# openai/tiktoken

Measured on AMD Instinct MI355X. Metric: GB/s text encoded (o200k_base-shaped vocab, 1 GiB corpus per GPU), bit-exact vs CoreBPE restatement, higher is better.
Workload: dtype u8; 1 GPU; o200k_shaped encode_ordinary_batch, 1024 MiB synthetic web-text per GPU (tkc_generate mix=1, seed 0x5EED0003), 318404 docs on rank 0, inputs resident in HBM, packed u32 output; encoding=o200k_shaped, pat_str_runs_on=hand-written scanners, bytes_per_gpu=1073741824, docs_rank0=318404, rccl_ranks=0, devices_visible=1, pieces_rank0=162498410, parallelism=doc-sharded x1

## Files before the change

### tiktoken_amd/csrc/tk_api.hip

```cpp
#include <hip/hip_runtime.h>
#include <dlfcn.h>
#include <rccl/rccl.h>
#include <stdio.h>
#include <stdlib.h>
#include <string.h>

#include <chrono>
#include <functional>
#include <algorithm>
#include <array>
#include <atomic>
#include <map>
#include <memory>
#include <mutex>
#include <string>
#include <thread>
#include <utility>
#include <vector>

#include "../../include/tiktoken_amd.h"
#include "tk_decode.h"
#include "tk_offsets.h"
#include "tk_rows.h"
#include "tk_train.h"
// ... 78 lines not shown
        std::swap(p, o.p);
        return *this;
    }
    ~HostResult() { if (p) tk_free(p); }
    T* release() { return std::exchange(p, nullptr); }
    operator T*() const { return p; }
};

struct KernelStat {
    double ms = 0;
    uint64_t launches = 0;
};

#define TK_NAUX 6
#define TK_NSET 4

#define TK_WORK_BUFS(X)                                                                                                                                  \
    X(text_al) X(tile_sum) X(wide_ws) X(scan_sums) X(row_base) X(brk) X(docb) X(cand) X(ss) X(si) X(starts) X(blockcnt) X(pstart) X(res) X(staging)     \
    X(listB) X(listC) X(counters) X(total) X(g_id) X(g_rk) X(g_nx) X(g_pv) X(g_lv) X(tile_np) X(tile_nt) X(mt_keys) X(mtab) X(movf) X(mcnt) X(wbin)       \
    X(deferred) X(big) X(rx_spec) X(rx_gst) X(rx_lnk) X(rx_exit) X(merge_work) X(find)
struct WorkSet {
    Pinned<uint32_t> h_counters;
    Pinned<uint64_t> h_total;
    Stream sb;
    Event ev_front;
    Event ev_cnt;
    Event ev_tot;
    Event ev_done;
    Event ev_fork, ev_join[TK_NAUX];
#define X(name) Buf name;
    TK_WORK_BUFS(X)
#undef X
    uint64_t bytes() const {
        uint64_t t = 0;
#define X(name) t += name.cap;
        TK_WORK_BUFS(X)
#undef X
        return t;
    }
};
#define TK_GROW (-1000)
#define TK_RESYNC (-1001)
#define TK_SPEC_HIT (-1002)
#ifndef TK_MT_DIV
#define TK_MT_DIV 128
#endif
// ... 35 lines not shown
    uint32_t ovf_base = 0;
    uint32_t ovf_cap = 0;
    bool optimistic = false;
};

static TkMiss miss_of(WorkSet& w, const ChunkJob& job) { return TkMiss{w.mtab.as<TkMissTab>(), w.movf.as<TkMissOvf>(), job.ovf_base, w.mcnt.as<uint8_t>()}; }

struct tk_core {
    int device = 0;
    Stream stream;
    Stream aux[TK_NAUX];
    Stream cs_h2d, cs_d2h;
    Pinned<void> stage[2];
    Event ev_stage[2];
    TkHostTables H;
    TkTables D;
    Buf t_stage1, t_stage2, t_bmp, t_byte_tab, t_short, t_mid, t_dec, t_piece, t_piece_off, t_tok_bytes, t_pair, t_pair2, t_byte_rank, t_xl, t_xfilter, t_spec_bytes, t_spec_off, t_spec_id, t_spec_head;
    uint32_t spec_max_len = 0;
    bool has_rx = false;
    bool has_rx_fb = false;
    TkRxCompiled rx_fb;
    uint64_t st_fallbacks = 0;
    uint64_t st_regrown = 0;
    uint64_t st_resynced = 0;
    bool defer_sync = false;
    uint32_t defer_ppm = 1u << 12;
    TkRxDev rx{};
    Buf t_rx_ins, t_rx_sets, t_rx_ranges, t_rx_first, t_rx_s1, t_rx_s2, t_rx_dtrans, t_rx_dascii, t_rx_ds1, t_rx_ds2;
    int rx_form = TK_RX_FORM_PROGRAM;
    std::mutex mu;
    WorkSet ws[TK_NSET];
    Buf text, doc_off, out_tokens, out_tok_off, allowed, tok_bases;
    Buf disallowed;
    bool find_on = false;
    uint64_t find_hit = ~0ull;
    uint64_t st_find_launches = 0;
    hipStream_t back_for = nullptr;
    struct BackChoice {
        hipStream_t s[3];
        int n;
    };
    std::map<hipStream_t, BackChoice> back_known;
    bool back_probed = false;
    hipStream_t back_s[3] = {};
    int n_back = 0;
    Pinned<uint32_t> h_probe;
// ... 159 lines not shown
    }
    int ndev = 0;
    if (hipGetDeviceCount(&ndev) != hipSuccess || ndev <= 0)
        return fail(TK_RUNTIME_ERROR, "no HIP device available: tiktoken_amd has no CPU path");
    if (device < 0 || device >= ndev) return fail(TK_VALUE_ERROR, "device ordinal out of range");
    struct Destroy {
        void operator()(tk_core* core) const { tk_destroy(core); }
    };
    std::unique_ptr<tk_core, Destroy> owner(new tk_core());
    tk_core* c = owner.get();
    c->device = device;
    std::string err = tk_build_tables(ranks_blob, ranks_off, ranks_ids, n_ranks, spec_blob, spec_off, spec_ids, n_spec, pat_str, &c->H);
    if (!err.empty()) return fail(TK_VALUE_ERROR, err);
    if (hipSetDevice(device) != hipSuccess) return fail(TK_RUNTIME_ERROR, "hipSetDevice failed");
    if (c->stream.create() != hipSuccess) return fail(TK_RUNTIME_ERROR, "hipStreamCreate failed");
    for (int i = 0; i < TK_NAUX; ++i)
        if (c->aux[i].create() != hipSuccess) return fail(TK_RUNTIME_ERROR, "hipStreamCreate failed");
    for (WorkSet& w : c->ws) {
        if (w.sb.create() != hipSuccess) return fail(TK_RUNTIME_ERROR, "hipStreamCreate failed");
        for (Event* e : {&w.ev_front, &w.ev_cnt, &w.ev_tot, &w.ev_done, &w.ev_fork})
            if (e->create() != hipSuccess) return fail(TK_RUNTIME_ERROR, "hipEventCreate failed");
        for (int i = 0; i < TK_NAUX; ++i)
            if (w.ev_join[i].create() != hipSuccess) return fail(TK_RUNTIME_ERROR, "hipEventCreate failed");
        if (w.h_counters.alloc(2 * TK_CNT_N * 4 + 64, hipHostMallocDefault) != hipSuccess || w.h_total.alloc(64, hipHostMallocDefault) != hipSuccess)
            return fail(TK_RUNTIME_ERROR, "hipHostMalloc failed");
    }
    const TkHostTables& H = c->H;
    auto upload_rx = [&](const TkRxCompiled& X) -> int {
        TRY(upload(c->t_rx_ins, X.ins.data(), X.ins.size() * sizeof(TkRxIns)));
        TRY(upload(c->t_rx_sets, X.sets.data(), X.sets.size() * sizeof(TkRxSet)));
        TRY(upload(c->t_rx_ranges, X.ranges.data(), X.ranges.size() * 4));
        TRY(upload(c->t_rx_first, X.first.data(), X.first.size() * 4));
        TRY(upload(c->t_rx_s1, tk_rx_props_stage1(), 0x1100));
        TRY(upload(c->t_rx_s2, tk_rx_props_stage2(), (size_t)tk_rx_props_blocks() * 256));
        c->rx = TkRxDev{c->t_rx_ins.as<TkRxIns>(), c->t_rx_sets.as<TkRxSet>(), c->t_rx_ranges.as<uint32_t>(), c->t_rx_s1.as<uint8_t>(),
                        c->t_rx_s2.as<uint8_t>(), (uint32_t)X.ins.size(), (uint32_t)X.sets.size(), (uint32_t)X.ranges.size() / 2,
                        c->t_rx_first.as<uint32_t>(), (uint32_t)X.first.size() / 8, nullptr, nullptr, nullptr, nullptr, 0u, 0u, 0u};
        c->rx_form = TK_RX_FORM_PROGRAM;
        const char* want = getenv("TIKTOKEN_AMD_RX_MATCHER");
        if (X.has_dfa() && !(want && !strcmp(want, "program"))) {
            std::vector<uint16_t> tr(X.dfa_trans);
            tr.resize((tr.size() + 1) & ~(size_t)1, 0);
            TRY(upload(c->t_rx_dtrans, tr.data(), tr.size() * 2));
            TRY(upload(c->t_rx_dascii, X.dfa_ascii.data(), 384));
            TRY(upload(c->t_rx_ds1, X.dfa_s1.data(), X.dfa_s1.size() * 2));
            TRY(upload(c->t_rx_ds2, X.dfa_s2.data(), X.dfa_s2.size()));
            c->rx.dfa_trans = c->t_rx_dtrans.as<uint16_t>();
            c->rx.dfa_ascii = c->t_rx_dascii.as<uint8_t>();
// ... 161 lines not shown
    uint64_t g = (items + per_block - 1) / per_block;
    if (g < 1) g = 1;
    if (g > cap) g = cap;
    return (uint32_t)g;
}

template <int MODE>
static void launch_front(tk_core* c, const ChunkJob& job, dim3 grid, hipStream_t s, uint32_t* deferred, int internal_dbg) {
    const ChunkAsk& a = job.ask;
    const FrontArgs& f = job.front;
    auto go = [&](auto* kernel) {
        hipLaunchKernelGGL(kernel, grid, dim3(256), 0, s, c->D, a.d_text, a.n, a.base, f.brk, f.docb, f.ss, f.si, f.out, f.mt, f.mt_mask, deferred, f.gapb, f.dbg | internal_dbg);
    };
    auto of_pattern = [&](auto pat) {
        if (f.ss) go(tk_k_front<decltype(pat)::value, true, MODE>);
        else go(tk_k_front<decltype(pat)::value, false, MODE>);
    };
    if (f.pat_id == TK_PAT_R50K) of_pattern(std::integral_constant<int, TK_PAT_R50K>{});
    else if (f.pat_id == TK_PAT_CL100K) of_pattern(std::integral_constant<int, TK_PAT_CL100K>{});
    else if (f.pat_id == TK_PAT_O200K) of_pattern(std::integral_constant<int, TK_PAT_O200K>{});
    else of_pattern(std::integral_constant<int, TK_PAT_GENERIC>{});
}

static int scan_u32(tk_core* c, WorkSet& w, hipStream_t s, uint32_t* a, uint64_t n, uint64_t* total_out) {
    if (n <= 2 * (uint64_t)TK_SCAN_BLOCK) {
        TRY(timed(c, s, "tk_k_scan_small", [&] { hipLaunchKernelGGL(tk_k_scan_small, dim3(1), dim3(TK_SCAN_THREADS), 0, s, a, n, total_out); }));
        return TK_OK;
    }
    const uint64_t nb = (n + TK_SCAN_BLOCK - 1) / TK_SCAN_BLOCK;
    TRY(ensure(w.scan_sums, (nb + 2) * 4));
    uint32_t* sums = w.scan_sums.as<uint32_t>();
    TRY(timed(c, s, "tk_k_scan_sums", [&] { hipLaunchKernelGGL(tk_k_scan_sums, dim3((uint32_t)nb), dim3(TK_SCAN_THREADS), 0, s, a, n, sums); }));
    TRY(timed(c, s, "tk_k_scan_small", [&] { hipLaunchKernelGGL(tk_k_scan_small, dim3(1), dim3(TK_SCAN_THREADS), 0, s, sums, nb, total_out); }));
    TRY(timed(c, s, "tk_k_scan_apply", [&] { hipLaunchKernelGGL(tk_k_scan_apply, dim3((uint32_t)nb), dim3(TK_SCAN_THREADS), 0, s, a, n, sums); }));
    return TK_OK;
}

static int rx_failure(const uint32_t* counters, uint64_t base) {
    const std::string at = std::to_string(base + (uint64_t)(~counters[TK_CNT_RXPOS]));
    if (counters[TK_CNT_ERR] & TK_RX_ERR_STACK)
        return fail(TK_VALUE_ERROR, "pat_str: a repeated group needs more backtracking state than the matcher keeps (piece at byte " + at +
                                        " of the batch); make the group possessive, e.g. (?:...)++");
    return fail(TK_VALUE_ERROR, "pat_str: backtrack limit exceeded at byte " + at +
                                    " of the batch (nested quantifiers; the reference's fancy-regex gives up after 1 000 000 backtracks as well)");
}

struct RxPairs {
    const uint64_t nwords;
    explicit RxPairs(uint64_t n) : nwords((n + 31) / 32) {}
    uint64_t bytes() const { return 2 * (nwords + 2) * 4; }
    uint32_t* gap(const Buf& pair) const { return pair.as<uint32_t>() + nwords + 2; }
    static std::array<Buf*, 3> of(WorkSet& w) { return {&w.rx_spec, &w.rx_gst, &w.rx_lnk}; }
};

static int rx_split(tk_core* c, WorkSet& w, const ChunkJob& job, hipStream_t s) {
    const uint8_t* d_text = job.ask.d_text;
    const uint64_t n = job.ask.n, nwords = (n + 31) / 32;
// ... 118 lines not shown
    TRY(ensure(w.big, (1 + 3 * TK_BIGCOPY_CAP) * 4));
    TkClearArgs clr;
    clr.n = 0;
    auto clear = [&](Buf& b, uint64_t bytes, uint32_t v) -> int {
        TRY(ensure(b, bytes));
        clr.p[clr.n] = b.as<uint4>();
        clr.n16[clr.n] = (bytes + 15) / 16;
        clr.v[clr.n] = v;
        ++clr.n;
        return TK_OK;
    };
    TRY(clear(w.brk, (nwords + 2) * 4, 0u));
    TRY(clear(w.counters, TK_CNT_N * 4, 0u));
    TRY(clear(w.big, 4, 0u));
    TRY(clear(w.merge_work, 16 * TKM_WORK_STRIDE * 4, 0u));
    TRY(clear(w.total, 32, 0u));
    uint32_t* find_docb = nullptr;
    const bool docs_in_place = n > 0 && !single_piece && ask.d_tok_off != nullptr;
    TRY(ensure(w.row_base, (ntiles + 4) * 4));
    if (docs_in_place) TRY(clear(w.row_base, (ntiles + 2) * 4, 0xFFFFFFFFu));
    TRY(clear(w.tile_sum, ntiles + 16, 0xFFFFFFFFu));
    FrontArgs& f = job.front;
    if (job.ovf_base) {
        TRY(clear(w.mt_keys, sizeof(TkMissKey) * job.ovf_base, 0xFFFFFFFFu));
        job.mt = w.mt_keys.as<TkMissKey>();
    }
    f.pat_id = T.pat.generic() ? TK_PAT_GENERIC : T.pattern;
    f.brk = w.brk.as<uint32_t>();
    f.out = TkFrontOut{w.starts.as<uint32_t>(), w.tile_np.as<uint32_t>(), w.res.as<uint32_t>(), w.tile_sum.as<uint8_t>(), miss_of(w, job), job.ovf_cap, w.listC.as<uint32_t>(), w.counters.as<uint32_t>()};
    f.mt = (c->dbg & TK_DBG_NO_MT) ? (TkMissKey*)nullptr : job.mt;
    f.mt_mask = (1u << job.mt_bits) - 1u;
    f.dbg = (c->dbg & ~TK_DBG_INTERNAL) | (pretok_only ? TK_DBG_STARTS_ONLY : 0);
    if (n > 0 && !single_piece) {
        if (ask.use_special) {
            for (Buf* b : {&w.docb, &w.cand}) TRY(clear(*b, (nwords + 4) * 4, 0u));
            for (Buf* b : {&w.ss, &w.si}) TRY(clear(*b, (nwords + 2) * 4, 0u));
            f.docb = w.docb.as<uint32_t>();
            f.ss = w.ss.as<uint32_t>();
            f.si = w.si.as<uint32_t>();
        }
        if (c->find_on && !pretok_only) {
            job.find = true;
            TRY(clear(w.find, 16, 0xFFFFFFFFu));
            if (!f.docb) TRY(clear(w.docb, (nwords + 4) * 4, 0u));
            find_docb = w.docb.as<uint32_t>();
        }
        if (c->has_rx) {
// ... 27 lines not shown
        }
        if (c->has_rx) TRY(rx_split(c, w, job, s));
        TRY(ensure(w.deferred, 2 * (ntiles + 2) * 4));
        TRY(timed(c, s, "tk_k_front", [&] {
            launch_front<TKF_MODE_TILE>(c, job, dim3((uint32_t)ntiles), s, w.deferred.as<uint32_t>(), (c->has_rx && !(c->dbg & TK_DBG_SCANNERS)) ? TK_DBG_HARD_ONLY : 0);
        }));
    } else if (n > 0) {
        hipLaunchKernelGGL(tk_k_chunk_clear, dim3(1), dim3(256), 0, s, clr);
        clr.n = 0;
        TRY(timed(c, s, "tk_k_single_front", [&] { hipLaunchKernelGGL(tk_k_single_front, dim3(1), dim3(64), 0, s, T, d_text, (uint32_t)n, f.out, ask.kind == ChunkKind::SinglePieceNoLookup ? 1 : 0); }));
    }
    if (clr.n) hipLaunchKernelGGL(tk_k_chunk_clear, dim3(1), dim3(256), 0, s, clr);
    HIPCHK(hipEventRecord(w.ev_front, s));
    return TK_OK;
}

static int piece_starts(tk_core* c, WorkSet& w, const ChunkJob& job, hipStream_t s, uint64_t* count_out) {
    const uint64_t n = job.ask.n, nwords = (n + 31) / 32, nblk = (nwords + 255) / 256;
    uint32_t *starts = w.starts.as<uint32_t>(), *blockcnt = w.blockcnt.as<uint32_t>();
    uint64_t P = 0;
    TRY(ensure(w.pstart, 16));
    if (n > 0) {
        TRY(timed(c, s, "tk_k_count", [&] { hipLaunchKernelGGL(tk_k_count, dim3((uint32_t)nblk), dim3(256), 0, s, starts, nwords, blockcnt); }));
        TRY(timed(c, s, "tk_k_scan_small", [&] { hipLaunchKernelGGL(tk_k_scan_small, dim3(1), dim3(TK_SCAN_THREADS), 0, s, blockcnt, nblk, w.total.as<uint64_t>()); }));
        HIPCHK(hipMemcpyAsync(&P, w.total.p, 8, hipMemcpyDeviceToHost, s));
        HIPCHK(hipStreamSynchronize(s));
        if (w.h_counters[TK_CNT_ERR] & (TK_RX_ERR_GAP | TK_RX_ERR_STACK | TK_RX_ERR_LIMIT)) return rx_failure(w.h_counters, job.ask.base);
        TRY(ensure(w.pstart, (P + 2) * 4));
        TRY(timed(c, s, "tk_k_emit", [&] {
            hipLaunchKernelGGL(tk_k_emit, dim3((uint32_t)nblk), dim3(256), 0, s, starts, nwords, blockcnt, w.pstart.as<uint32_t>(), P, n, job.front.gapb);
        }));
    } else {
        HIPCHK(hipMemsetAsync(w.pstart.p, 0, 4, s));
    }
    *count_out = P;
    return TK_OK;
}

static int stage_back(tk_core* c, WorkSet& w, ChunkJob& job, hipStream_t s, hipEvent_t prev_tot = nullptr) {
    const TkTables& T = c->D;
    const ChunkAsk& ask = job.ask;
    const uint64_t n = ask.n, ntiles = job.ntiles;
    const uint8_t* d_text = ask.d_text;
    uint32_t *d_out = ask.d_out, *counters = w.counters.as<uint32_t>();
    uint32_t *res = w.res.as<uint32_t>(), *stg = w.staging.as<uint32_t>();
    const TkMiss data = miss_of(w, job);
    uint32_t *tile_np = w.tile_np.as<uint32_t>(), *tile_nt = w.tile_nt.as<uint32_t>();
// ... 79 lines not shown
            if (rounds) {
                TRY(timed(c, s, "tk_k_merge_rounds", [&] {
                    hipLaunchKernelGGL(tk_k_merge_rounds, dim3(grid_for(nC, 1, 1024)), dim3(TKB_THREADS), 0, s, T, d_text, w.listC.as<uint32_t>(),
                                       (uint32_t)nC, w.g_id.as<uint32_t>(), w.g_rk.as<uint32_t>(), w.g_nx.as<uint32_t>(), w.g_pv.as<uint32_t>(),
                                       data, stg);
                }));
            }
            if (rounds && n >= TK_WIDE_MIN) {
                TRY(ensure(w.wide_ws, sizeof(TkWideWs)));
                HIPCHK(hipMemsetAsync(w.wide_ws.p, 0, sizeof(TkWideWs), s));
                TRY(timed(c, s, "tk_k_merge_rounds_wide", [&] {
                    hipLaunchKernelGGL(tk_k_merge_rounds_wide, dim3(TK_WIDE_BLOCKS), dim3(TKB_THREADS), 0, s, T, d_text, w.listC.as<uint32_t>(),
                                       (uint32_t)nC, w.g_id.as<uint32_t>(), w.g_rk.as<uint32_t>(), w.g_nx.as<uint32_t>(), w.g_pv.as<uint32_t>(),
                                       data, stg, w.wide_ws.as<TkWideWs>());
                }));
            }
            TRY(timed(c, s, "tk_k_merge_long", [&] {
                hipLaunchKernelGGL(tk_k_merge_long, dim3(grid_for(nC, 4, 8192)), dim3(256), 0, s, T, d_text, w.listC.as<uint32_t>(), (uint32_t)nC,
                                   w.g_id.as<uint32_t>(), w.g_rk.as<uint32_t>(), w.g_nx.as<uint32_t>(), w.g_pv.as<uint32_t>(),
                                   w.g_lv.as<uint64_t>(), data, stg, rounds ? 1 : 0);
            }));
        }
    }
    const bool small_rows = n < (8u << 20);
    if (encode) {
        TRY(timed(c, s, "tk_k_count_tiles", [&] {
            if (small_rows) hipLaunchKernelGGL(tk_k_count_tiles<1>, dim3(grid_for(ntiles, 4, 2048)), dim3(256), 0, s, ntiles, tile_np, res, data, tile_nt,
                               w.total.as<unsigned long long>());
            else hipLaunchKernelGGL(tk_k_count_tiles<TKP_ROWS_COUNT>, dim3(grid_for(ntiles, 4, 2048)), dim3(256), 0, s, ntiles, tile_np, res, data, tile_nt,
                               w.total.as<unsigned long long>());
        }));
        TRY(scan_u32(c, w, s, tile_nt, ntiles, w.total.as<uint64_t>()));
    } else {
        HIPCHK(hipMemsetAsync(w.total.p, 0, 32, s));
    }
    if (prev_tot) HIPCHK(hipStreamWaitEvent(s, prev_tot, 0));
    hipLaunchKernelGGL(tk_k_advance, dim3(1), dim3(64), 0, s, c->tok_bases.as<unsigned long long>(), job.index, w.total.as<uint64_t>());
    HIPCHK(hipEventRecord(w.ev_tot, s));
    if (encode) {
        TRY(timed(c, s, "tk_k_place", [&] {
            const bool docs_in_place = !ask.single_piece() && ask.d_tok_off != nullptr;
            const TkPlaceDocs docs{ask.d_doc_off, ask.base, n, ask.n_docs, w.row_base.as<uint32_t>(), w.starts.as<uint32_t>(), w.total.as<uint64_t>(), docs_in_place ? ask.d_tok_off : (uint64_t*)nullptr};
            hipLaunchKernelGGL(tk_k_place<TKP_ROWS_PLACE>, dim3(grid_for(ntiles, 4, 6144)), dim3(256), 0, s, ntiles, tile_np, tile_nt, res, data, stg, d_out, tok_base, w.big.as<uint32_t>(), docs);
        }));
    }
    if (encode && n > TK_BIGCOPY)
        hipLaunchKernelGGL(tk_k_bigcopy, dim3(1024), dim3(256), 0, s, w.big.as<uint32_t>(), stg, d_out, tok_base);
    if (!front_only && ask.d_tok_off && (n == 0 || ask.single_piece())) {
        TRY(timed(c, s, "tk_k_docoff", [&] {
            hipLaunchKernelGGL(tk_k_docoff, dim3(grid_for(ask.n_docs + 1, 16, 4096)), dim3(256), 0, s, ask.n_docs, ask.d_doc_off, ask.base, n, w.starts.as<uint32_t>(), tile_nt, res, data,
                               (n > 0 && !ask.single_piece()) ? w.row_base.as<uint32_t>() : (const uint32_t*)nullptr, w.total.as<uint64_t>(), tok_base, ask.d_tok_off);
        }));
    }
    HIPCHK(hipMemcpyAsync(w.h_total, w.total.p, 16, hipMemcpyDeviceToHost, s));
    if (job.find) HIPCHK(hipMemcpyAsync(w.h_total + 2, w.find.p, 8, hipMemcpyDeviceToHost, s));
    HIPCHK(hipMemcpyAsync(w.h_counters + TK_CNT_N, counters, TK_CNT_N * 4, hipMemcpyDeviceToHost, s));
    HIPCHK(hipEventRecord(w.ev_done, s));
    c->st_long += nC;
    return TK_OK;
}

static int chunk_finish(tk_core* c, WorkSet& w, const ChunkJob& job, uint64_t* n_tokens_out) {
    HIPCHK(hipEventSynchronize(w.ev_done));
    if (job.find && w.h_total[2] != ~0ull) {
        c->find_hit = w.h_total[2];
        return TK_SPEC_HIT;
    }
    const uint32_t* hb = w.h_counters + TK_CNT_N;
    uint64_t nB = 0;
    for (int b = 0; b < TK_NBIN; ++b) {
        nB += hb[TK_CNT_BIN0 + b];
        if ((c->dbg & TK_DBG_VERBOSE) && hb[TK_CNT_BIN0 + b]) fprintf(stderr, "bin %d (%u..%u bytes): %u pieces\n", b, tk_bin_lo(b), tk_bin_hi(b), hb[TK_CNT_BIN0 + b]);
    }
    if (hb[TK_CNT_ERR] & (TK_RX_ERR_GAP | TK_RX_ERR_STACK | TK_RX_ERR_LIMIT)) return rx_failure(hb, job.ask.base);
    if (hb[TK_CNT_ERR]) return fail(TK_RUNTIME_ERROR, "internal error in the front kernel (scanner list overflow, code " + std::to_string(hb[TK_CNT_ERR]) + ")");
    if (job.optimistic) {
        if (hb[TK_CNT_DEFER2]) {
            c->defer_sync = true;
            return TK_RESYNC;
        }
        const uint32_t ppm = (uint32_t)std::min<uint64_t>(((uint64_t)hb[TK_CNT_DEFER] << 20) / (job.ntiles ? job.ntiles : 1), 1u << 20);
        c->defer_ppm = std::max(ppm, c->defer_ppm / 4);
    }
    if (hb[TK_CNT_OVF] > job.ovf_cap && !job.ask.piece_starts()) {
        c->ovf_full = true;
        return TK_GROW;
    }
    c->st_bytes += job.ask.n;
    c->st_pieces += w.h_total[1];
    c->st_tokens += w.h_total[0];
    c->st_medium += nB;
    c->st_chunks += 1;
    *n_tokens_out = w.h_total[0];
    return TK_OK;
}

static int run_chunk(tk_core* c, hipStream_t s, const ChunkAsk& ask, uint64_t* n_out) {
    WorkSet& w = c->ws[0];
    ChunkJob job;
    TRY(ensure(c->tok_bases, 64));
    HIPCHK(hipMemsetAsync(c->tok_bases.p, 0, 16, s));
    TRY(stage_front(c, w, job, s, ask));
    if (ask.piece_starts()) {
        TRY(stage_deferred(c, w, job, s));
        return piece_starts(c, w, job, s, n_out);
    }
    TRY(stage_back(c, w, job, s));
    return chunk_finish(c, w, job, n_out);
}

static int prepare_mask(tk_core* c, hipStream_t s, Buf& mask, const uint32_t* ids, uint64_t n, bool* any) {
    const TkHostTables& H = c->H;
    std::vector<uint8_t> a(H.spec_id.size() + 16, 0);
    *any = false;
    for (size_t k = 0; k < H.spec_id.size(); ++k)
// ... 2022 lines not shown
    if (launches_out) *launches_out = it->second.launches;
    return TK_OK;
}
extern "C" void tk_last_stats(tk_core* c, uint64_t* n_bytes, uint64_t* n_pieces, uint64_t* n_tokens, uint64_t* n_docs,
                              uint64_t* n_medium, uint64_t* n_long) {
    if (!c) return;
    if (n_bytes) *n_bytes = c->st_bytes;
    if (n_pieces) *n_pieces = c->st_pieces;
    if (n_tokens) *n_tokens = c->st_tokens;
    if (n_docs) *n_docs = c->st_docs;
    if (n_medium) *n_medium = c->st_medium;
    if (n_long) *n_long = c->st_long;
}
extern "C" uint64_t tk_stat(tk_core* c, const char* name) {
    if (!c || !name) return 0;
    const std::string k(name);
    if (k == "front_wgs_per_cu") return TKF_OCC;
    if (k == "compute_units") return c->n_cu;
    if (k == "chunks") return c->st_chunks;
    if (k == "small_launches") return c->st_small_launches;
    if (k == "small_calls") return c->st_small_calls;
    if (k == "mid_calls") return c->st_mid_calls;
    if (k == "back_streams") return (uint64_t)c->n_back;
    if (k == "resynced") return c->st_resynced;
    if (k == "spec_find_launches") return c->st_find_launches;
    if (k == "regrown") return c->st_regrown;
    if (k == "workspace_bytes") {
        uint64_t t = 0;
        for (auto& w : c->ws) t += w.bytes();
        return t;
    }
    if (k == "deferred_count") return c->ws[0].h_counters ? c->ws[0].h_counters[TK_CNT_N + TK_CNT_DEFER] : 0;
    if (k.rfind("deferred_tile_", 0) == 0) {
        uint32_t v = 0;
        const uint64_t i = strtoull(k.c_str() + 14, nullptr, 10);
        if (c->ws[0].deferred.p && (i + 1) * 4 <= c->ws[0].deferred.cap && hipMemcpy(&v, c->ws[0].deferred.as<uint32_t>() + i, 4, hipMemcpyDeviceToHost) != hipSuccess) v = 0xFFFFFFFFu;
        return v;
    }
    if (k == "fallbacks") return c->st_fallbacks;
    if (k == "host_front_us") return (uint64_t)c->host_us[0];
    if (k == "host_back_us") return (uint64_t)c->host_us[1];
    if (k == "host_back_wait_us") return (uint64_t)c->host_us[2];
    if (k == "host_finish_us") return (uint64_t)c->host_us[3];
    if (k == "host_tail_us") return (uint64_t)c->host_us[4];
    if (k == "host_total_us") return (uint64_t)c->host_us[5];
    if (k == "chunk_bytes") return c->chunk_bytes;
// ... 22 lines not shown
```

### tiktoken_amd/csrc/tk_fused.h

```cpp
#pragma once
#include <type_traits>

#include "tk_chunk.h"
#include "tk_kernels.h"

#define TKF_NONE 0xFFFFFFFFu
#define TK_MERGE_REDO 0xFFFFFFFFu
#define TK_BIGCOPY 4096
#define TK_BIGCOPY_CAP 1024
#define TKF_CHAIN_END 0xFFFFFFFFFFFFFFFFull
#define TKF_CONT_CAP 768
#define TKF_CONT_CAP_FAST 768
#define TKF_SLOW_CAP 8
#define TKF_WALK_BUDGET 32u
#define TKF_MODE_TILE 0
#define TKF_MODE_STARTS 1
#define TKF_MODE_GIVEN 2
#define TKF_BATCH 896
#define TKF_BL 14
#define TKF_CAP 4096
#define TKF_TAIL_NMISS (TKF_CAP - 1)
#define TKF_TAIL_NGAP (TKF_CAP - 2)
#define TKF_TAIL_REFS (TKF_CAP - 3)

// ... 1691 lines not shown
                if (rk != TK_RANK_MAX) {
                    const uint32_t i = i0 + j * 64u + (uint32_t)lane;
                    data.put(i, 1u, rk);
                    if (i < ovf_base) mt[i].w2 = TK_EMPTY_KEY;
#pragma unroll
                    for (int jj = 0; jj < 4; ++jj)
                        if (j == (uint32_t)jj) len[jj] = 0u;
                }
            }
        }
#pragma unroll
        for (int j = 0; j < 4; ++j) {
            const uint32_t bin = tk_miss_bin_of_len(len[j]);
#pragma unroll
            for (int b = 0; b < TK_NBIN; ++b) nb[b] += (uint32_t)__popcll(__ballot(bin == (uint32_t)b));
        }
    }
    if (lane == 0) {
#pragma unroll
        for (int b = 0; b < TK_NBIN; ++b) wbin[(uint32_t)b * nwaves + wave] = nb[b];
    }
}

__global__ __launch_bounds__(256) void tk_k_binfill(TkTables T, const uint8_t* __restrict__ text, TkMiss data, const TkMissKey* __restrict__ mt, uint32_t ovf_cap,
                                                    const uint32_t* __restrict__ wscan, uint32_t* __restrict__ listB, uint32_t* __restrict__ counters) {
    const uint32_t ovf_base = data.ovf_base;
    const int lane = threadIdx.x & 63;
    const uint32_t wave = (blockIdx.x * 256u + threadIdx.x) >> 6;
    const uint32_t nwaves = gridDim.x * 4u;
    const uint32_t E = tk_miss_entries(counters, ovf_base, ovf_cap);
    const uint32_t per = ((E + nwaves - 1u) / nwaves + 63u) & ~63u;
    const uint64_t lo64 = (uint64_t)wave * per;
    const uint32_t lo = lo64 < E ? (uint32_t)lo64 : E, hi = lo64 + per < E ? (uint32_t)(lo64 + per) : E;
    uint32_t at[TK_NBIN];
#pragma unroll
    for (int b = 0; b < TK_NBIN; ++b) at[b] = wscan[(uint32_t)b * nwaves + wave];
    if (wave == 0 && lane < TK_NBIN) {
        counters[TK_CNT_BIN0 + lane] = wscan[(uint32_t)(lane + 1) * nwaves] - wscan[(uint32_t)lane * nwaves];
        counters[TK_CNT_BOFF0 + lane] = wscan[(uint32_t)lane * nwaves];
    }
    for (uint32_t i0 = lo; i0 < hi; i0 += 64) {
        const uint32_t i = i0 + (uint32_t)lane;
        uint32_t start, len = tk_miss_len(data, mt, i, hi, start);
        if (i >= ovf_base && tk_miss_may_be_token(T, len) && tk_lookup_text_piece(T, text, start, len) != TK_RANK_MAX) len = 0u;
        const uint32_t bin = tk_miss_bin_of_len(len);
#pragma unroll
        for (int b = 0; b < TK_NBIN; ++b) {
            const uint64_t m = __ballot(bin == (uint32_t)b);
            if (bin == (uint32_t)b) listB[at[b] + (uint32_t)__popcll(m & ((1ull << lane) - 1ull))] = i;
            at[b] += (uint32_t)__popcll(m);
        }
    }
}

__device__ __forceinline__ void tk_put_result(const TkMiss& data, uint32_t i, uint32_t cnt, uint32_t tok) { data.put(i, cnt, tok); }
template <int NMAX, int THREADS>
__global__ __launch_bounds__(THREADS) void tk_k_merge_llane(TkTables T, const uint8_t* __restrict__ text, const uint32_t* __restrict__ listB,
                                                             const uint32_t* __restrict__ counters, int bin, TkMiss data,
                                                             uint32_t* __restrict__ staging) {
    const uint32_t count = counters[TK_CNT_BIN0 + bin];
    const uint32_t* __restrict__ list = listB + counters[TK_CNT_BOFF0 + bin];
    __shared__ uint32_t s_id[NMAX * THREADS];
    __shared__ uint32_t s_rk[NMAX * THREADS];
    uint32_t* id = s_id + threadIdx.x;
    uint32_t* rk = s_rk + threadIdx.x;
    for (uint32_t it = blockIdx.x * THREADS + threadIdx.x; it < count; it += gridDim.x * THREADS) {
// ... 1235 lines not shown
            uint32_t cb[16];
            bool escape = false;
#pragma unroll
            for (int j = 0; j < 16; ++j) {
                if (k0 + (uint32_t)j >= kp) rv[j] = TK_RES_GAP;
                const bool flagged = rv[j] != TK_RES_GAP && (rv[j] & TK_RES_FLAG), in_tab = flagged && (rv[j] & ~TK_RES_FLAG) < data.ovf_base;
                cb[j] = data.cnt8[in_tab ? (rv[j] & ~TK_RES_FLAG) : 0u];
                if (flagged && (!in_tab || cb[j] == 255u)) escape = true;
                else sum += flagged ? cb[j] : (rv[j] != TK_RES_GAP ? 1u : 0u);
            }
            if (escape) {
#pragma unroll
                for (int j = 0; j < 16; ++j) {
                    const bool flagged = rv[j] != TK_RES_GAP && (rv[j] & TK_RES_FLAG), in_tab = flagged && (rv[j] & ~TK_RES_FLAG) < data.ovf_base;
                    if (flagged && (!in_tab || cb[j] == 255u)) sum += TKD_COUNT(data.head(rv[j] & ~TK_RES_FLAG)[2]);
                }
            }
        }
        const uint64_t v = inside ? row_run + tk_row16_sum(sum) : total[0];
        if (have && sl == 0) tok_off[d] = tok_base_global + v;
    }
}

__global__ void tk_k_advance(unsigned long long* __restrict__ tok_bases, uint32_t k, const uint64_t* __restrict__ total) {
    if (blockIdx.x == 0 && threadIdx.x == 0) tok_bases[k + 1] = tok_bases[k] + total[0];
}

__global__ void tk_k_single_front(TkTables T, const uint8_t* __restrict__ text, uint32_t n, TkFrontOut out, int no_lookup) {
    if (blockIdx.x || threadIdx.x) return;
    out.tile_np[0] = 1;
    const uint32_t r = (no_lookup && n > 1u) ? TK_RANK_MAX : tk_lookup_text_piece(T, text, 0, n);
    out.res[TKF_TAIL_NGAP] = 0;
    out.res[TKF_TAIL_NMISS] = r != TK_RANK_MAX ? 0u : 1u;
    if (r != TK_RANK_MAX) {
        out.res[0] = r;
    } else {
        out.res[TKF_TAIL_REFS] = out.data.ovf_base;
        out.res[0] = TK_RES_FLAG | out.data.ovf_base;
        *(uint4*)&out.data.ovf[0].start = make_uint4(0u, n, 0u, 0u);
        out.counters[TK_CNT_OVF] = 1;
        if (n > TK_GLANE_MAX) tk_append_tree(out.listC, out.counters, out.data.ovf_base, 0, n);
    }
}

#define TK_SMALL_MAX 2048
#define TK_SMALL_PIECE 24
#define TK_SMALL_LONG 256
#define TK_SMALL_NO_LONG 0x80000000u
#define TK_SMALL_HDR 4
struct TkSmallAcc {
// ... 195 lines not shown
```

### tiktoken_amd/csrc/tk_kernels.h

```cpp
#pragma once
#include <hip/hip_runtime.h>

#include "tk_device.h"
#include "tk_scan.h"
#include "tk_special.h"

#define TK_TILE 3840

#define TK_NBIN 9
#define TK_GLANE_MAX 1024
__host__ __device__ inline uint32_t tk_bin_hi(int b) {
    const uint32_t hi[TK_NBIN] = {16, 24, 32, 48, 64, 128, 256, 512, TK_GLANE_MAX};
    return hi[b];
}
__host__ __device__ inline uint32_t tk_bin_lo(int b) { return b == 0 ? 2u : tk_bin_hi(b - 1) + 1; }
__device__ __forceinline__ int tk_bin_of(uint32_t len) {
    int b = 0;
#pragma unroll
    for (int i = 0; i < TK_NBIN - 1; ++i) b += len > tk_bin_hi(i);
    return b;
}

enum {
    TK_CNT_B = 0, TK_CNT_C = 1, TK_CNT_CBYTES = 2, TK_CNT_CLEVELS = 3, TK_CNT_DUP = 4, TK_CNT_COLL = 5, TK_CNT_ERR = 6, TK_CNT_DEFER = 7,
// ... 212 lines not shown
        const uint32_t w0 = wi + j;
        if (w0 + 1 > TK2_NSEG + 1) return kind == TKB_HARD ? ~0ull : 0ull;
        return sh ? ((bm[kind][w0] >> sh) | (bm[kind][w0 + 1] << (64u - sh))) : bm[kind][w0];
    }
    __device__ __forceinline__ uint32_t limit() const { return lim; }
};

__device__ __forceinline__ uint64_t tk_piece_end_slow(TkWin2Acc* acc, uint64_t p, TkPat pat) {
    uint64_t e = tk_piece_end(*acc, p, pat);
    if (e <= p) e = tk_next_char(*acc, p);
    return e;
}
__global__ __launch_bounds__(256) void tk_k_count(const uint32_t* __restrict__ starts, uint64_t nwords, uint32_t* __restrict__ blockcnt) {
    __shared__ uint32_t sh[8];
    uint64_t w = blockIdx.x * 256ull + threadIdx.x;
    uint32_t c = w < nwords ? __popc(starts[w]) : 0;
    c = tk_wave_sum_u32(c);
    if ((threadIdx.x & 63) == 0) sh[threadIdx.x >> 6] = c;
    __syncthreads();
    if (threadIdx.x == 0) blockcnt[blockIdx.x] = sh[0] + sh[1] + sh[2] + sh[3];
}

#define TK_SCAN_THREADS 256
__global__ __launch_bounds__(TK_SCAN_THREADS) void tk_k_scan_small(uint32_t* __restrict__ a, uint64_t n, uint64_t* __restrict__ total_out) {
    constexpr int NW = TK_SCAN_THREADS / 64;
    __shared__ uint32_t wsum[NW];
    __shared__ uint64_t carry_sh;
    if (threadIdx.x == 0) carry_sh = 0;
    __syncthreads();
    const int lane = threadIdx.x & 63, wid = threadIdx.x >> 6;
    constexpr int E = 16;
    for (uint64_t base = 0; base < n; base += TK_SCAN_THREADS * E) {
        const uint64_t i0 = base + (uint64_t)threadIdx.x * E;
        uint32_t v[E], mine = 0;
#pragma unroll
        for (int j = 0; j < E; ++j) {
            v[j] = i0 + j < n ? a[i0 + j] : 0;
            mine += v[j];
        }
        const uint32_t inc = tk_wave_scan_u32(mine, lane);
        if (lane == 63) wsum[wid] = inc;
        __syncthreads();
        uint32_t wbase = 0, tot = 0;
#pragma unroll
        for (int w = 0; w < NW; ++w) {
            if (w < wid) wbase += wsum[w];
            tot += wsum[w];
        }
        const uint64_t carry = carry_sh;
        uint32_t run = (uint32_t)(carry + wbase + inc - mine);
#pragma unroll
        for (int j = 0; j < E; ++j) {
            if (i0 + j < n) a[i0 + j] = run;
            run += v[j];
        }
        __syncthreads();
        if (threadIdx.x == 0) carry_sh = carry + tot;
        __syncthreads();
    }
    if (threadIdx.x == 0) total_out[0] = carry_sh;
}

#define TK_SCAN_BLOCK 4096
__global__ __launch_bounds__(TK_SCAN_THREADS) void tk_k_scan_sums(const uint32_t* __restrict__ a, uint64_t n, uint32_t* __restrict__ sums) {
    constexpr int NW = TK_SCAN_THREADS / 64, E = TK_SCAN_BLOCK / TK_SCAN_THREADS;
    __shared__ uint32_t wsum[NW];
    const uint64_t i0 = (uint64_t)blockIdx.x * TK_SCAN_BLOCK + (uint64_t)threadIdx.x * E;
    uint32_t mine = 0;
#pragma unroll
    for (int j = 0; j < E; ++j) mine += i0 + j < n ? a[i0 + j] : 0u;
    mine = tk_wave_sum_u32(mine);
    if ((threadIdx.x & 63) == 0) wsum[threadIdx.x >> 6] = mine;
    __syncthreads();
    if (threadIdx.x == 0) {
        uint32_t t = 0;
#pragma unroll
        for (int w = 0; w < NW; ++w) t += wsum[w];
        sums[blockIdx.x] = t;
    }
}
__global__ __launch_bounds__(TK_SCAN_THREADS) void tk_k_scan_apply(uint32_t* __restrict__ a, uint64_t n, const uint32_t* __restrict__ bases) {
    constexpr int NW = TK_SCAN_THREADS / 64, E = TK_SCAN_BLOCK / TK_SCAN_THREADS;
    __shared__ uint32_t wsum[NW];
    const int lane = threadIdx.x & 63, wid = threadIdx.x >> 6;
    const uint64_t i0 = (uint64_t)blockIdx.x * TK_SCAN_BLOCK + (uint64_t)threadIdx.x * E;
    uint32_t v[E], mine = 0;
#pragma unroll
    for (int j = 0; j < E; ++j) {
        v[j] = i0 + j < n ? a[i0 + j] : 0u;
        mine += v[j];
    }
    const uint32_t inc = tk_wave_scan_u32(mine, lane);
    if (lane == 63) wsum[wid] = inc;
    __syncthreads();
    uint32_t wbase = 0;
    for (int w = 0; w < wid; ++w) wbase += wsum[w];
    uint32_t run = bases[blockIdx.x] + wbase + inc - mine;
#pragma unroll
    for (int j = 0; j < E; ++j) {
        if (i0 + j < n) a[i0 + j] = run;
        run += v[j];
    }
}

__global__ __launch_bounds__(256) void tk_k_emit(const uint32_t* __restrict__ starts, uint64_t nwords, const uint32_t* __restrict__ blockpre,
                                                 uint32_t* __restrict__ pstart, uint64_t P, uint64_t n, const uint32_t* __restrict__ gapb) {
    __shared__ uint32_t sh[8];
    uint64_t w = blockIdx.x * 256ull + threadIdx.x;
    uint32_t v = w < nwords ? starts[w] : 0;
    uint32_t tot;
    uint32_t ex = tk_block_exscan_256(__popc(v), &tot, sh);
    uint64_t o = (uint64_t)blockpre[blockIdx.x] + ex;
    while (v) {
        uint32_t b = __ffs(v) - 1;
        v &= v - 1;
        pstart[o++] = (uint32_t)(w * 32 + b) | ((gapb && ((gapb[w] >> b) & 1u)) ? 0x80000000u : 0u);
    }
    if (blockIdx.x == 0 && threadIdx.x == 0) pstart[P] = (uint32_t)n;
}
```

Measured before the change: 176.1 GB/s.

## Fold chunk-end bookkeeping into scan kernels and skip redundant miss-key clears

The per-chunk tok_bases advance and the device-to-host copies of totals, find result and counters now happen inside the last scan kernel. They write straight into coherent, mapped pinned host memory, which removes a separate advance launch and three async memcpys per chunk. The miss-key table is now reset to empty by tk_k_binfill as it reads each slot, so the next chunk can skip its full memset when the buffer was not reallocated. The risk is that counters and totals are captured earlier in the stream than before, and that correctness now depends on binfill visiting every slot it needs to clean.

```diff
diff --git a/tiktoken_amd/csrc/tk_api.hip b/tiktoken_amd/csrc/tk_api.hip
--- a/tiktoken_amd/csrc/tk_api.hip
+++ b/tiktoken_amd/csrc/tk_api.hip
@@ -124,6 +124,9 @@
 struct WorkSet {
     Pinned<uint32_t> h_counters;
     Pinned<uint64_t> h_total;
+    uint32_t* d_counters1 = nullptr;
+    uint64_t* d_total = nullptr;
+    uint64_t keys_clean = 0, keys_next = 0;
     Stream sb;
     Event ev_front;
     Event ev_cnt;
@@ -205,6 +208,7 @@
     TkRxCompiled rx_fb;
     uint64_t st_fallbacks = 0;
     uint64_t st_regrown = 0;
+    uint64_t st_key_skips = 0;
     uint64_t st_resynced = 0;
     bool defer_sync = false;
     uint32_t defer_ppm = 1u << 12;
@@ -410,8 +414,15 @@
             if (e->create() != hipSuccess) return fail(TK_RUNTIME_ERROR, "hipEventCreate failed");
         for (int i = 0; i < TK_NAUX; ++i)
             if (w.ev_join[i].create() != hipSuccess) return fail(TK_RUNTIME_ERROR, "hipEventCreate failed");
-        if (w.h_counters.alloc(2 * TK_CNT_N * 4 + 64, hipHostMallocDefault) != hipSuccess || w.h_total.alloc(64, hipHostMallocDefault) != hipSuccess)
+        if (w.h_counters.alloc(2 * TK_CNT_N * 4 + 64, hipHostMallocCoherent | hipHostMallocMapped) != hipSuccess ||
+            w.h_total.alloc(64, hipHostMallocCoherent | hipHostMallocMapped) != hipSuccess)
             return fail(TK_RUNTIME_ERROR, "hipHostMalloc failed");
+        memset(w.h_counters, 0, 2 * TK_CNT_N * 4 + 64);
+        memset(w.h_total, 0, 64);
+        uint32_t* dc = nullptr;
+        if (hipHostGetDevicePointer((void**)&dc, w.h_counters, 0) != hipSuccess || hipHostGetDevicePointer((void**)&w.d_total, w.h_total, 0) != hipSuccess)
+            return fail(TK_RUNTIME_ERROR, "hipHostGetDevicePointer failed");
+        w.d_counters1 = dc + TK_CNT_N;
     }
     const TkHostTables& H = c->H;
     auto upload_rx = [&](const TkRxCompiled& X) -> int {
@@ -619,17 +630,19 @@
     else of_pattern(std::integral_constant<int, TK_PAT_GENERIC>{});
 }
 
-static int scan_u32(tk_core* c, WorkSet& w, hipStream_t s, uint32_t* a, uint64_t n, uint64_t* total_out) {
+static int scan_u32(tk_core* c, WorkSet& w, hipStream_t s, uint32_t* a, uint64_t n, uint64_t* total_out, const TkChunkEnd& end = TkChunkEnd{}, hipEvent_t wait_first = nullptr) {
     if (n <= 2 * (uint64_t)TK_SCAN_BLOCK) {
-        TRY(timed(c, s, "tk_k_scan_small", [&] { hipLaunchKernelGGL(tk_k_scan_small, dim3(1), dim3(TK_SCAN_THREADS), 0, s, a, n, total_out); }));
+        if (wait_first) HIPCHK(hipStreamWaitEvent(s, wait_first, 0));
+        TRY(timed(c, s, "tk_k_scan_small", [&] { hipLaunchKernelGGL(tk_k_scan_small, dim3(1), dim3(TK_SCAN_THREADS), 0, s, a, n, total_out, end); }));
         return TK_OK;
     }
     const uint64_t nb = (n + TK_SCAN_BLOCK - 1) / TK_SCAN_BLOCK;
     TRY(ensure(w.scan_sums, (nb + 2) * 4));
     uint32_t* sums = w.scan_sums.as<uint32_t>();
     TRY(timed(c, s, "tk_k_scan_sums", [&] { hipLaunchKernelGGL(tk_k_scan_sums, dim3((uint32_t)nb), dim3(TK_SCAN_THREADS), 0, s, a, n, sums); }));
-    TRY(timed(c, s, "tk_k_scan_small", [&] { hipLaunchKernelGGL(tk_k_scan_small, dim3(1), dim3(TK_SCAN_THREADS), 0, s, sums, nb, total_out); }));
-    TRY(timed(c, s, "tk_k_scan_apply", [&] { hipLaunchKernelGGL(tk_k_scan_apply, dim3((uint32_t)nb), dim3(TK_SCAN_THREADS), 0, s, a, n, sums); }));
+    TRY(timed(c, s, "tk_k_scan_small", [&] { hipLaunchKernelGGL(tk_k_scan_small, dim3(1), dim3(TK_SCAN_THREADS), 0, s, sums, nb, total_out, TkChunkEnd{}); }));
+    if (wait_first) HIPCHK(hipStreamWaitEvent(s, wait_first, 0));
+    TRY(timed(c, s, "tk_k_scan_apply", [&] { hipLaunchKernelGGL(tk_k_scan_apply, dim3((uint32_t)nb), dim3(TK_SCAN_THREADS), 0, s, a, n, sums, end); }));
     return TK_OK;
 }
 
@@ -794,7 +807,13 @@
     TRY(clear(w.tile_sum, ntiles + 16, 0xFFFFFFFFu));
     FrontArgs& f = job.front;
     if (job.ovf_base) {
-        TRY(clear(w.mt_keys, sizeof(TkMissKey) * job.ovf_base, 0xFFFFFFFFu));
+        const void* had = w.mt_keys.p;
+        TRY(ensure(w.mt_keys, sizeof(TkMissKey) * job.ovf_base));
+        const bool clean = w.mt_keys.p == had && w.keys_clean >= job.ovf_base;
+        if (clean) c->st_key_skips += 1;
+        else TRY(clear(w.mt_keys, sizeof(TkMissKey) * job.ovf_base, 0xFFFFFFFFu));
+        w.keys_next = clean ? w.keys_clean : job.ovf_base;
+        w.keys_clean = 0;
         job.mt = w.mt_keys.as<TkMissKey>();
     }
     f.pat_id = T.pat.generic() ? TK_PAT_GENERIC : T.pattern;
@@ -868,7 +887,7 @@
     TRY(ensure(w.pstart, 16));
     if (n > 0) {
         TRY(timed(c, s, "tk_k_count", [&] { hipLaunchKernelGGL(tk_k_count, dim3((uint32_t)nblk), dim3(256), 0, s, starts, nwords, blockcnt); }));
-        TRY(timed(c, s, "tk_k_scan_small", [&] { hipLaunchKernelGGL(tk_k_scan_small, dim3(1), dim3(TK_SCAN_THREADS), 0, s, blockcnt, nblk, w.total.as<uint64_t>()); }));
+        TRY(timed(c, s, "tk_k_scan_small", [&] { hipLaunchKernelGGL(tk_k_scan_small, dim3(1), dim3(TK_SCAN_THREADS), 0, s, blockcnt, nblk, w.total.as<uint64_t>(), TkChunkEnd{}); }));
         HIPCHK(hipMemcpyAsync(&P, w.total.p, 8, hipMemcpyDeviceToHost, s));
         HIPCHK(hipStreamSynchronize(s));
         if (w.h_counters[TK_CNT_ERR] & (TK_RX_ERR_GAP | TK_RX_ERR_STACK | TK_RX_ERR_LIMIT)) return rx_failure(w.h_counters, job.ask.base);
@@ -994,6 +1013,8 @@
             }));
         }
     }
+    const TkChunkEnd end{c->tok_bases.as<unsigned long long>(), job.index, w.total.as<uint64_t>(), job.find ? w.find.as<uint64_t>() : (const uint64_t*)nullptr,
+                         counters, w.d_total, w.d_counters1};
     const bool small_rows = n < (8u << 20);
     if (encode) {
         TRY(timed(c, s, "tk_k_count_tiles", [&] {
@@ -1002,12 +1023,12 @@
             else hipLaunchKernelGGL(tk_k_count_tiles<TKP_ROWS_COUNT>, dim3(grid_for(ntiles, 4, 2048)), dim3(256), 0, s, ntiles, tile_np, res, data, tile_nt,
                                w.total.as<unsigned long long>());
         }));
-        TRY(scan_u32(c, w, s, tile_nt, ntiles, w.total.as<uint64_t>()));
+        TRY(scan_u32(c, w, s, tile_nt, ntiles, w.total.as<uint64_t>(), end, prev_tot));
     } else {
         HIPCHK(hipMemsetAsync(w.total.p, 0, 32, s));
-    }
-    if (prev_tot) HIPCHK(hipStreamWaitEvent(s, prev_tot, 0));
-    hipLaunchKernelGGL(tk_k_advance, dim3(1), dim3(64), 0, s, c->tok_bases.as<unsigned long long>(), job.index, w.total.as<uint64_t>());
+        if (prev_tot) HIPCHK(hipStreamWaitEvent(s, prev_tot, 0));
+        hipLaunchKernelGGL(tk_k_advance, dim3(1), dim3(64), 0, s, end);
+    }
     HIPCHK(hipEventRecord(w.ev_tot, s));
     if (encode) {
         TRY(timed(c, s, "tk_k_place", [&] {
@@ -1024,9 +1045,6 @@
                                (n > 0 && !ask.single_piece()) ? w.row_base.as<uint32_t>() : (const uint32_t*)nullptr, w.total.as<uint64_t>(), tok_base, ask.d_tok_off);
         }));
     }
-    HIPCHK(hipMemcpyAsync(w.h_total, w.total.p, 16, hipMemcpyDeviceToHost, s));
-    if (job.find) HIPCHK(hipMemcpyAsync(w.h_total + 2, w.find.p, 8, hipMemcpyDeviceToHost, s));
-    HIPCHK(hipMemcpyAsync(w.h_counters + TK_CNT_N, counters, TK_CNT_N * 4, hipMemcpyDeviceToHost, s));
     HIPCHK(hipEventRecord(w.ev_done, s));
     c->st_long += nC;
     return TK_OK;
@@ -1063,6 +1081,7 @@
     c->st_tokens += w.h_total[0];
     c->st_medium += nB;
     c->st_chunks += 1;
+    if (job.mt && TKF_STOP_AFTER == 0) w.keys_clean = w.keys_next;
     *n_tokens_out = w.h_total[0];
     return TK_OK;
 }
@@ -3131,6 +3150,7 @@
     if (k == "small_calls") return c->st_small_calls;
     if (k == "mid_calls") return c->st_mid_calls;
     if (k == "back_streams") return (uint64_t)c->n_back;
+    if (k == "key_clears_skipped") return c->st_key_skips;
     if (k == "resynced") return c->st_resynced;
     if (k == "spec_find_launches") return c->st_find_launches;
     if (k == "regrown") return c->st_regrown;
diff --git a/tiktoken_amd/csrc/tk_fused.h b/tiktoken_amd/csrc/tk_fused.h
--- a/tiktoken_amd/csrc/tk_fused.h
+++ b/tiktoken_amd/csrc/tk_fused.h
@@ -1737,7 +1737,7 @@
     }
 }
 
-__global__ __launch_bounds__(256) void tk_k_binfill(TkTables T, const uint8_t* __restrict__ text, TkMiss data, const TkMissKey* __restrict__ mt, uint32_t ovf_cap,
+__global__ __launch_bounds__(256) void tk_k_binfill(TkTables T, const uint8_t* __restrict__ text, TkMiss data, TkMissKey* __restrict__ mt, uint32_t ovf_cap,
                                                     const uint32_t* __restrict__ wscan, uint32_t* __restrict__ listB, uint32_t* __restrict__ counters) {
     const uint32_t ovf_base = data.ovf_base;
     const int lane = threadIdx.x & 63;
@@ -1756,7 +1756,19 @@
     }
     for (uint32_t i0 = lo; i0 < hi; i0 += 64) {
         const uint32_t i = i0 + (uint32_t)lane;
-        uint32_t start, len = tk_miss_len(data, mt, i, hi, start);
+        uint32_t start = 0, len = 0;
+        if (i < hi && i < ovf_base) {
+            uint4* slot = (uint4*)&mt[i];
+            const uint4 a = slot[0], b = slot[1];
+            const unsigned long long w2 = (unsigned long long)b.z | ((unsigned long long)b.w << 32);
+            if (w2 != TK_EMPTY_KEY) {
+                start = (uint32_t)w2;
+                len = (w2 >> 63) ? ((uint32_t)(w2 >> 32) & 0x7FFFFFFFu) : (uint32_t)(w2 >> 56);
+            }
+            if ((a.x & a.y & a.z & a.w & b.x & b.y & b.z & b.w) != 0xFFFFFFFFu) slot[0] = slot[1] = make_uint4(0xFFFFFFFFu, 0xFFFFFFFFu, 0xFFFFFFFFu, 0xFFFFFFFFu);
+        } else {
+            len = tk_miss_len(data, mt, i, hi, start);
+        }
         if (i >= ovf_base && tk_miss_may_be_token(T, len) && tk_lookup_text_piece(T, text, start, len) != TK_RANK_MAX) len = 0u;
         const uint32_t bin = tk_miss_bin_of_len(len);
 #pragma unroll
@@ -3038,10 +3050,6 @@
     }
 }
 
-__global__ void tk_k_advance(unsigned long long* __restrict__ tok_bases, uint32_t k, const uint64_t* __restrict__ total) {
-    if (blockIdx.x == 0 && threadIdx.x == 0) tok_bases[k + 1] = tok_bases[k] + total[0];
-}
-
 __global__ void tk_k_single_front(TkTables T, const uint8_t* __restrict__ text, uint32_t n, TkFrontOut out, int no_lookup) {
     if (blockIdx.x || threadIdx.x) return;
     out.tile_np[0] = 1;
diff --git a/tiktoken_amd/csrc/tk_kernels.h b/tiktoken_amd/csrc/tk_kernels.h
--- a/tiktoken_amd/csrc/tk_kernels.h
+++ b/tiktoken_amd/csrc/tk_kernels.h
@@ -258,7 +258,26 @@
 }
 
 #define TK_SCAN_THREADS 256
-__global__ __launch_bounds__(TK_SCAN_THREADS) void tk_k_scan_small(uint32_t* __restrict__ a, uint64_t n, uint64_t* __restrict__ total_out) {
+
+struct TkChunkEnd {
+    unsigned long long* tok_bases;
+    uint32_t k;
+    const uint64_t* total;
+    const uint64_t* find;
+    const uint32_t* counters;
+    uint64_t* h_total;
+    uint32_t* h_counters;
+};
+__device__ __forceinline__ void tk_chunk_end(const TkChunkEnd& e, uint64_t tokens) {
+    e.tok_bases[e.k + 1] = e.tok_bases[e.k] + tokens;
+    e.h_total[0] = tokens;
+    e.h_total[1] = e.total[1];
+    if (e.find) e.h_total[2] = e.find[0];
+    for (int i = 0; i < TK_CNT_N; ++i) e.h_counters[i] = e.counters[i];
+    __threadfence_system();
+}
+
+__global__ __launch_bounds__(TK_SCAN_THREADS) void tk_k_scan_small(uint32_t* __restrict__ a, uint64_t n, uint64_t* __restrict__ total_out, TkChunkEnd end) {
     constexpr int NW = TK_SCAN_THREADS / 64;
     __shared__ uint32_t wsum[NW];
     __shared__ uint64_t carry_sh;
@@ -294,7 +313,10 @@
         if (threadIdx.x == 0) carry_sh = carry + tot;
         __syncthreads();
     }
-    if (threadIdx.x == 0) total_out[0] = carry_sh;
+    if (threadIdx.x == 0) {
+        total_out[0] = carry_sh;
+        if (end.tok_bases) tk_chunk_end(end, carry_sh);
+    }
 }
 
 #define TK_SCAN_BLOCK 4096
@@ -315,7 +337,7 @@
         sums[blockIdx.x] = t;
     }
 }
-__global__ __launch_bounds__(TK_SCAN_THREADS) void tk_k_scan_apply(uint32_t* __restrict__ a, uint64_t n, const uint32_t* __restrict__ bases) {
+__global__ __launch_bounds__(TK_SCAN_THREADS) void tk_k_scan_apply(uint32_t* __restrict__ a, uint64_t n, const uint32_t* __restrict__ bases, TkChunkEnd end) {
     constexpr int NW = TK_SCAN_THREADS / 64, E = TK_SCAN_BLOCK / TK_SCAN_THREADS;
     __shared__ uint32_t wsum[NW];
     const int lane = threadIdx.x & 63, wid = threadIdx.x >> 6;
@@ -337,6 +359,11 @@
         if (i0 + j < n) a[i0 + j] = run;
         run += v[j];
     }
+    if (end.tok_bases && blockIdx.x + 1 == gridDim.x && threadIdx.x == 0) tk_chunk_end(end, end.total[0]);
+}
+
+__global__ void tk_k_advance(TkChunkEnd end) {
+    if (blockIdx.x == 0 && threadIdx.x == 0) tk_chunk_end(end, end.total[0]);
 }
 
 __global__ __launch_bounds__(256) void tk_k_emit(const uint32_t* __restrict__ starts, uint64_t nwords, const uint32_t* __restrict__ blockpre,
```

Measured after the change: 176.1 GB/s (median of 2 runs). Within noise of the previous version (-0.0%).
